# snarkify/sirius

Hardware: AMD Instinct MI355X
Metric: IVC fold-steps/s (CycleFold IVC::next hot path, Poseidon-shaped synthetic trace, 2^k rows) (higher is better)
Workload: dtype u256 (modular; 9 x 29-bit / 8 x 32-bit limbs)

## Files before the change

### sirius_amd/csrc/msm.h

```cpp
#pragma once
#include "curve.cuh"
#include "devrt.h"
#include "glv.cuh"
#include "stripes.h"
#include "tuning.h"

#include <cstdlib>

namespace srs {
namespace msm {

constexpr int WBITS = 16;
constexpr int NWIN = 16;
constexpr int NWIN_COMPACT = 8;
constexpr uint32_t PAY_ENDO = 1u << 30;
constexpr uint32_t NBUCKET = 1u << (WBITS - 1);

constexpr uint32_t SORT_THREADS = 1024;
constexpr uint32_t SORT_TILE_MIN = 8192;
constexpr uint32_t SORT_TARGET_BLOCKS = 256;
constexpr uint32_t SEG = 128, SEG_BUCKETS = NBUCKET / SEG;
constexpr uint32_t SORT_TILE2 = 8192;
constexpr uint64_t TWO_PASS_MIN_SLOTS = 1ull << 23;
constexpr uint32_t PLAN_THREADS = 1024;
constexpr uint32_t ACC_THREADS = 256;
constexpr uint32_t ACC_L0_LOG = 4, ACC_L0 = 1u << ACC_L0_LOG;
constexpr uint32_t ACC_L1_LOG = 3, ACC_L1 = 1u << ACC_L1_LOG;
constexpr uint32_t FINAL_THREADS = 256;
constexpr uint32_t FINAL_FANIN = 512;
constexpr int MAX_LEVELS = 8;
constexpr uint32_t RED_ROWS = 256;
constexpr uint32_t RED_COLS = NBUCKET / RED_ROWS;
constexpr uint32_t RED_THREADS = 4 * RED_COLS;
constexpr uint32_t ACC1_QUAD_MAX = 1u << 17;
constexpr uint32_t BATCH_ARGS = 16;
constexpr uint32_t LANDING_SLOTS = 16;
constexpr uint32_t NORM_G = 16;
constexpr uint32_t SLOT_LOG = 6;
constexpr uint32_t SLOT_L0_MIN_LOG = 2, SLOT_L0_MAX_LOG = 16;
constexpr int WBITS_W = 20;
constexpr int NWIN_W = 13;
constexpr uint32_t NSEG_W = 16;
constexpr uint32_t WIDE_THREADS = 256, WIDE_PER = 2, WIDE_TILE = WIDE_THREADS * WIDE_PER;
constexpr uint32_t WIDE_MIN_KEY_LOG = 23;
constexpr uint32_t WIDE_MIN_N_LOG = 23;

static_assert(RED_ROWS == 256 && RED_COLS == 128, "k_rowcol lane layout");
static_assert(NBUCKET % PLAN_THREADS == 0, "k_plan tiling");

inline bool expect_ovf_initial() { return tuning::get_or(tuning::MSM_EXPECT_OVF, 1) != 0; }

struct Key {
    int curve = 0;
    size_t len = 0;
    size_t global_len = 0;
    uint32_t rank = 0, world = 1;
    bool compact = false;
    bool compact_scalars = false;
    affine_t *table = nullptr;
    affine_t *table_w = nullptr;
    uint64_t stat_slot_sets = 0, stat_hot_sets = 0, stat_redo = 0, stat_other_sets = 0;
    uint64_t last_entries = 0;
    uint64_t last_scalars = 0;

    Arena arena;
    void *h_result = nullptr;
    struct Landing { bool wide = false, slot_mode = false, ovf_on = false; uint32_t batch = 0; } landing[LANDING_SLOTS];
    xyzz_t *fold_buckets = nullptr;
    xyzz_t *slots = nullptr;
    size_t slots_pts = 0;
    uint8_t *used = nullptr;
    uint32_t *h_ovf = nullptr;
    uint32_t slot_s = 0;
    uint32_t seq = 0;
    bool commit_ovf = false;
    bool expect_ovf = expect_ovf_initial();
    uint32_t cold_streak = 0;
};

int choose_windows(Key &k);
void build_table(Key &k, hipStream_t stream);
size_t table_bytes(const Key &k);
void release(Key &k);
void generate_bases(Key &k, uint64_t seed, hipStream_t stream);

void read_bases(const Key &k, affine_t *out_dev, hipStream_t stream);

size_t count_off_curve(const Key &k, hipStream_t stream);

size_t workspace_bytes(uint32_t n_max, uint32_t batch);

void run(Key &k, const fe_t *const *scalars_dev, const uint32_t *n_host, uint32_t batch, int is_mont,
         hipStream_t stream, xyzz_t *result_host);

enum Fold { FOLD_NONE = 0, FOLD_FIRST = 1, FOLD_MIDDLE = 2, FOLD_LAST = 3 };
bool enqueue(Key &k, const fe_t *const *scalars_dev, const uint32_t *n_host, const uint32_t *base_host, uint32_t batch, int is_mont,
             hipStream_t stream, uint32_t slot, Fold fold = FOLD_NONE);
void finish(Key &k, uint32_t batch, uint32_t slot, bool launched, xyzz_t *result_host);
void reserve(Key &k, uint32_t n_max, uint32_t batch);
bool overflow_missed(const Key &k, uint32_t slot);
void note_commit(Key &k, const uint32_t *slots_used, uint32_t n_slots, uint64_t scalars);

}
}
```

### sirius_amd/csrc/msm.hip

```cpp
#define SRS_F29_CHAIN 1
#include "msm.h"
#include "tuning.h"
#include "curve29.cuh"
#include "prof.h"

#include <algorithm>
#include <cstdlib>
#include <numeric>
#include <vector>

namespace srs {
namespace msm {

__device__ __forceinline__ uint32_t upper_bucket(const uint32_t *__restrict__ tp, uint32_t t) {
    uint32_t lo = 0, hi = NBUCKET;
    while (hi - lo > 1) {
        uint32_t mid = (lo + hi) >> 1;
        if (tp[mid] <= t) lo = mid; else hi = mid;
    }
    return lo;
}

template <class C>
__global__ void k_table_step(const affine_t *__restrict__ prev, xyzz_t *__restrict__ tmp, uint32_t n, int nbits) {
// ... 1381 lines not shown
    const size_t ping_off = link ? (size_t)link->base[0][m] : (size_t)m * ping_stride;
    const size_t pong_off = link ? (size_t)link->base[1][m] : (size_t)m * pong_stride;
    const xyzz_t *B = (hdr[1] && !from_buckets) ? ((hdr[0] & 1u) ? ping + ping_off : pong + pong_off) : buckets + (size_t)m * NBUCKET;
    using E29 = Ec29<C>;
    xyzz_t *out = rc + (size_t)m * (RED_ROWS + RED_COLS);
    const bool is_row = blockIdx.x < RED_ROWS / 2;
    xyzz29_t acc;
    if (is_row) {
        const uint32_t hi = blockIdx.x * 2 + wave;
        const xyzz_t *src = B + (size_t)hi * RED_COLS + vl * SER;
        acc = E29::unpack(src[0]);
        xyzz_t nx = src[1];
        for (uint32_t j = 1; j < SER; ++j) {
            xyzz_t cur = nx;
            if (j + 1 < SER) nx = src[j + 1];
            acc = E29::add_quad(acc, E29::unpack(cur), q);
        }
    } else {
        const uint32_t lo = blockIdx.x - RED_ROWS / 2, sub = wave * 16 + vl;
        const xyzz_t *src = B + (size_t)(sub * SER) * RED_COLS + lo;
        acc = E29::unpack(src[0]);
        xyzz_t nx = src[RED_COLS];
        for (uint32_t j = 1; j < SER; ++j) {
            xyzz_t cur = nx;
            if (j + 1 < SER) nx = src[(size_t)(j + 1) * RED_COLS];
            acc = E29::add_quad(acc, E29::unpack(cur), q);
        }
    }
    for (unsigned d = 8; d >= 1; d >>= 1) {
        xyzz29_t o = shfl_down_point29(acc, 4 * d, 64);
        if (vl < d) acc = E29::add_quad(acc, o, q);
    }
    if (is_row) {
        if (lane == 0) out[blockIdx.x * 2 + wave] = E29::pack(acc);
        return;
    }
    if (wave == 1 && lane == 0) half[0] = E29::pack(acc);
    __syncthreads();
    if (wave == 0 && vl == 0) {
        acc = E29::add_quad(acc, E29::unpack(half[0]), q);
        if (q == 0) out[RED_ROWS + (blockIdx.x - RED_ROWS / 2)] = E29::pack(acc);
    }
}

template <class C>
__global__ void SRS_KERNEL_BOUNDS(RED_THREADS, 1)
    k_reduce_final(const xyzz_t *__restrict__ rc, xyzz_t *__restrict__ out) {
    constexpr uint32_t N = RED_COLS;
    using E29 = Ec29<C>;
    __shared__ xyzz29_t v[N];
    const uint32_t m = blockIdx.y, t = threadIdx.x >> 2, q = threadIdx.x & 3u, which = blockIdx.x;
    const xyzz_t *rows = rc + (size_t)m * (RED_ROWS + RED_COLS), *cols = rows + RED_ROWS;
    xyzz29_t x;
    if (which == 0) x = E29::add_quad(E29::unpack(rows[2 * t]), E29::unpack(rows[2 * t + 1]), q);
    else if (which == 1 || which == 3) x = E29::unpack(cols[t]);
    else x = E29::unpack(rows[2 * t + 1]);
    if (which < 2) {
        if (q == 0) v[t] = x;
        __syncthreads();
        for (uint32_t s = 1; s < N; s <<= 1) {
            const bool has = t + s < N;
            xyzz29_t o = has ? v[t + s] : E29::identity();
            __syncthreads();
            if (has) x = E29::add_quad(x, o, q);
            if (q == 0) v[t] = x;
            __syncthreads();
        }
        if (which == 0 && t == 0) x = E29::identity();
    }
    if (q == 0) v[t] = x;
    __syncthreads();
    for (uint32_t s = N >> 1; s >= 1; s >>= 1) {
        if (t < s) {
            x = E29::add_quad(x, v[t + s], q);
            if (q == 0) v[t] = x;
        }
        __syncthreads();
    }
    if (threadIdx.x == 0) out[(size_t)m * gridDim.x + which] = E29::pack(v[0]);
}

template <class C>
__global__ void SRS_KERNEL_BOUNDS(256, 1)
    k_wide_combine(const xyzz_t *__restrict__ in , xyzz_t *__restrict__ out ) {
    using E29 = Ec29<C>;
    const uint32_t which = threadIdx.x >> 6, lane = threadIdx.x & 63u, q = lane & 3u, vl = lane >> 2;
    xyzz29_t x = E29::unpack(in[vl * 4 + which]);
    if (which == 3) {
        for (uint32_t s = 1; s < NSEG_W; s <<= 1) {
            xyzz29_t o = shfl_down_point29(x, 4 * s, 64);
            if (vl + s < NSEG_W) x = E29::add_quad(x, o, q);
        }
        if (vl == 0) x = E29::identity();
    }
    for (unsigned d = NSEG_W / 2; d >= 1; d >>= 1) {
        xyzz29_t o = shfl_down_point29(x, 4 * d, 64);
        if (vl < d) x = E29::add_quad(x, o, q);
    }
    if (lane == 0) out[which] = E29::pack(x);
}

static inline uint32_t ceil_div(uint64_t a, uint64_t b) { return (uint32_t)((a + b - 1) / b); }

template <class C>
static void expand_windows(affine_t *table, uint32_t n, int nwin, int nbits, xyzz_t *tmp, hipStream_t stream) {
    for (int w = 1; w < nwin; ++w) {
        const affine_t *prev = table + (size_t)(w - 1) * n;
        affine_t *cur = table + (size_t)w * n;
        SRS_LAUNCH((k_table_step<C>), (ceil_div(n, 256)), (256), 0, stream, prev, tmp, n, nbits);
        SRS_LAUNCH((k_normalize<C>), (ceil_div(ceil_div(n, NORM_G), 128)), (128), 0, stream, (const xyzz_t *)tmp, cur, n);
    }
}

static bool wants_wide_table(size_t len) {
    static const int env_forced = [] { const char *e = std::getenv("SRS_MSM_WIDE"); return e ? std::atoi(e) : -1; }();
    const int forced = (int)tuning::get_or(tuning::MSM_WIDE, env_forced);
    if (forced == 0 || len == 0) return false;
    return forced == 1 || len >= ((size_t)1 << WIDE_MIN_KEY_LOG);
}

template <class C>
static void build_table_t(Key &k, hipStream_t stream) {
    const uint32_t n = (uint32_t)k.len;
    if (k.table_w) {
        SRS_HIP_CHECK(hipFree(k.table_w));
        k.table_w = nullptr;
    }
    if (n == 0) return;
    xyzz_t *tmp = nullptr;
    SRS_HIP_CHECK(hipMalloc((void **)&tmp, (size_t)n * sizeof(xyzz_t)));
    if (!k.compact && wants_wide_table(n) && hipMalloc((void **)&k.table_w, (size_t)n * NWIN_W * sizeof(affine_t)) != hipSuccess) {
        (void)hipGetLastError();
        k.table_w = nullptr;
    }
    if (k.table_w) {
        SRS_HIP_CHECK(hipMemcpyAsync(k.table_w, k.table, (size_t)n * sizeof(affine_t), hipMemcpyDeviceToDevice, stream));
        expand_windows<C>(k.table_w, n, NWIN_W, WBITS_W, tmp, stream);
        const size_t total_w = (size_t)n * NWIN_W;
        SRS_LAUNCH((k_table_form<C>), (ceil_div(total_w, 256)), (256), 0, stream, k.table_w, total_w);
    }
    const int nwin = k.compact ? NWIN_COMPACT : NWIN;
    expand_windows<C>(k.table, n, nwin, WBITS, tmp, stream);
    const size_t total = (size_t)n * nwin;
    SRS_LAUNCH((k_table_form<C>), (ceil_div(total, 256)), (256), 0, stream, k.table, total);
    SRS_HIP_CHECK(hipStreamSynchronize(stream));
    SRS_HIP_CHECK(hipFree(tmp));
}

template <class C>
static void generate_t(Key &k, uint64_t seed, hipStream_t stream) {
    const uint32_t n = (uint32_t)k.len;
    if (n == 0) return;
    xyzz_t *tmp = nullptr;
    SRS_HIP_CHECK(hipMalloc((void **)&tmp, (size_t)n * sizeof(xyzz_t)));
    SRS_LAUNCH((k_gen_bases<C>), (ceil_div(n, 128)), (128), 0, stream, tmp, n, seed, k.rank, k.world);
    SRS_LAUNCH((k_normalize<C>), (ceil_div(ceil_div(n, NORM_G), 128)), (128), 0, stream, (const xyzz_t *)tmp, k.table, n);
    SRS_HIP_CHECK(hipStreamSynchronize(stream));
    SRS_HIP_CHECK(hipFree(tmp));
}
void generate_bases(Key &k, uint64_t seed, hipStream_t stream) {
    if (k.curve == 0) generate_t<Bn256>(k, seed, stream); else generate_t<Grumpkin>(k, seed, stream);
}

size_t count_off_curve(const Key &k, hipStream_t stream) {
    if (k.len == 0) return 0;
    uint32_t *d_bad = nullptr, bad = 0;
    SRS_HIP_CHECK(hipMalloc((void **)&d_bad, sizeof(uint32_t)));
    SRS_HIP_CHECK(hipMemsetAsync(d_bad, 0, sizeof(uint32_t), stream));
    const uint32_t n = (uint32_t)k.len;
    if (k.curve == 0) SRS_LAUNCH((k_on_curve<Bn256>), (ceil_div(n, 256)), (256), 0, stream, (const affine_t *)k.table, n, d_bad);
    else SRS_LAUNCH((k_on_curve<Grumpkin>), (ceil_div(n, 256)), (256), 0, stream, (const affine_t *)k.table, n, d_bad);
    SRS_HIP_CHECK(hipMemcpyAsync(&bad, d_bad, sizeof(uint32_t), hipMemcpyDeviceToHost, stream));
    SRS_HIP_CHECK(hipStreamSynchronize(stream));
    (void)hipFree(d_bad);
    return bad;
}

void read_bases(const Key &k, affine_t *out_dev, hipStream_t stream) {
    if (k.len == 0) return;
    if (k.curve == 0) SRS_LAUNCH((k_table_unform<Bn256>), (ceil_div(k.len, 256)), (256), 0, stream, (const affine_t *)k.table, out_dev, k.len);
    else SRS_LAUNCH((k_table_unform<Grumpkin>), (ceil_div(k.len, 256)), (256), 0, stream, (const affine_t *)k.table, out_dev, k.len);
}

void build_table(Key &k, hipStream_t stream) {
    if (k.curve == 0) build_table_t<Bn256>(k, stream); else build_table_t<Grumpkin>(k, stream);
}

int choose_windows(Key &k) {
    k.compact = tuning::get_or(tuning::MSM_COMPACT, 0) == 1;
    if (k.compact && (uint64_t)NWIN_COMPACT * k.len > PAY_ENDO) {
        set_error("compact key (msm_compact = 1): 8 x " + std::to_string(k.len) + " table entries do not fit below the endomorphism flag (2^30)");
        throw DeviceError{4};
    }
    return k.compact ? NWIN_COMPACT : NWIN;
}
size_t table_bytes(const Key &k) {
    if (!k.table) return 0;
    return k.len * sizeof(affine_t) * ((k.compact ? NWIN_COMPACT : NWIN) + (k.table_w ? NWIN_W : 0));
}


static uint32_t l0_log_for(uint64_t M) {
    const int forced = (int)tuning::get_or(tuning::MSM_L0, 0);
    if (forced >= 1 && forced <= 7) return (uint32_t)forced;
    if (M < (1ull << 20)) return 2;
    if (M < (1ull << 22)) return 3;
    uint32_t lg = ACC_L0_LOG;
    while (lg < 7 && (M >> (lg + 1)) >= (5ull << 20)) ++lg;
    return lg;
}

static uint32_t acc1_quad_max() {
    const int64_t lg = tuning::get_or(tuning::MSM_QUAD_MAX, 0);
    return (lg >= 1 && lg <= 24) ? (1u << lg) : ACC1_QUAD_MAX;
}

static int levels_for(uint64_t parts) {
    int levels = 1;
    while (parts > FINAL_FANIN && levels < MAX_LEVELS) {
        parts = (parts + ACC_L1 - 1) / ACC_L1;
        ++levels;
    }
    return levels;
}

static bool use_two_pass(uint64_t M, uint32_t batch) {
    const int forced = (int)tuning::get_or(tuning::MSM_SORT, 0);
    if (forced == 1) return false;
    if (forced == 2) return true;
    return M * batch >= TWO_PASS_MIN_SLOTS;
}

static uint32_t slot_log() {
    const int64_t lg = tuning::get_or(tuning::MSM_SLOT_LOG, 0);
    return (lg >= 2 && lg <= 8) ? (uint32_t)lg : SLOT_LOG;
}
static uint32_t slot_want_cap() { return 4u; }

struct LevelShape {
    uint64_t M;
    int levels;
    size_t plan_stride;
    uint64_t cap0, cap1;
    uint32_t quad_max;
};
struct SetShape : LevelShape {
    bool two_pass;
    uint32_t tile, tiles;
};
struct NarrowShape : SetShape { uint32_t l0_log; };
struct SlotShape : SetShape { uint32_t S, nred; };
struct WideShape : LevelShape { uint32_t l0_log, T, tiles_g; };

static void sort_shape(SetShape &h, uint32_t n_max, uint32_t batch) {
    h.M = (uint64_t)n_max * NWIN;
    h.quad_max = acc1_quad_max();
    h.two_pass = use_two_pass(h.M, batch);
    h.tile = (uint32_t)((h.M * batch + SORT_TARGET_BLOCKS - 1) / SORT_TARGET_BLOCKS);
    h.tile = (h.tile + 1023u) & ~1023u;
    if (h.tile < SORT_TILE_MIN) h.tile = SORT_TILE_MIN;
    h.tiles = ceil_div(n_max, h.tile);
}
static NarrowShape narrow_shape(uint32_t n_max, uint32_t batch) {
    NarrowShape h;
    sort_shape(h, n_max, batch);
    h.l0_log = l0_log_for(h.M);
    h.levels = levels_for((h.M + (1ull << h.l0_log) - 1) >> h.l0_log);
    h.plan_stride = (size_t)(h.levels + 1) * (NBUCKET + 1) + 4;
    h.cap0 = (h.M >> h.l0_log) + NBUCKET + 1;
    h.cap1 = h.cap0 / ACC_L1 + NBUCKET + 1;
    return h;
}
static SlotShape slot_shape(uint32_t n_max, uint32_t batch) {
    SlotShape h;
    sort_shape(h, n_max, batch);
    const uint32_t lg = slot_log();
    h.S = 1u << lg;
    h.nred = (lg + 2) / 3;
    h.cap0 = std::min<uint64_t>((uint64_t)NBUCKET * h.S, (h.M >> SLOT_L0_MIN_LOG) + NBUCKET);
    h.cap1 = h.cap0 / ACC_L1 + NBUCKET + 1;
    h.levels = levels_for(h.cap0);
    h.plan_stride = (size_t)(h.levels + 2) * (NBUCKET + 1) + 4;
    return h;
}
static WideShape wide_shape(uint32_t n) {
    WideShape w;
    w.M = (uint64_t)n * NWIN_W;
    w.quad_max = acc1_quad_max();
    w.l0_log = l0_log_for(w.M);
    w.levels = levels_for((w.M + (1ull << w.l0_log) - 1) >> w.l0_log);
    w.plan_stride = (size_t)(w.levels + 1) * (NBUCKET + 1) + 4;
    w.cap0 = (w.M >> w.l0_log) + (uint64_t)NSEG_W * (NBUCKET + 1);
    w.cap1 = w.cap0 / ACC_L1 + (uint64_t)NSEG_W * (NBUCKET + 1);
    w.T = ceil_div(n, WIDE_TILE);
    w.tiles_g = SORT_TARGET_BLOCKS;
    return w;
}

struct Sizer {
    size_t used = 0;
    template <class T>
    T *take(size_t count) {
        used += Arena::pad(count * sizeof(T));
        return nullptr;
    }
};
template <class Walk>
static size_t sized(Walk walk) {
    Sizer s;
    walk(s);
    return s.used;
}
template <class Walk>
static auto carve(Arena &A, Walk walk) {
    const size_t need = sized(walk);
    A.reserve(need);
    A.reset();
    const auto bufs = walk(A);
    if (A.used != need) {
        set_error("internal: msm workspace: the arena walk and the sizer disagree");
        throw DeviceError{5};
    }
    return bufs;
}

struct SetBufs {
    xyzz_t *d_out, *ping, *pong, *rc;
    uint16_t *dig, *tb;
    uint32_t *sorted, *count, *cursor, *plan;
    uint16_t *gkey;
    uint32_t *gpay, *tile_hist;
};
struct NarrowBufs : SetBufs { xyzz_t *buckets; };
struct SlotBufs : SetBufs { xyzz_t *red_a, *red_b; };
template <class W>
static void take_set_head(W &A, const SetShape &h, uint32_t batch, SetBufs &b) {
    b.d_out = A.template take<xyzz_t>(3 * (size_t)batch);
    b.dig = A.template take<uint16_t>(h.M * batch);
    b.sorted = A.template take<uint32_t>(h.M * batch);
    b.count = A.template take<uint32_t>((size_t)NBUCKET * batch);
    b.cursor = A.template take<uint32_t>((size_t)NBUCKET * batch);
    b.plan = A.template take<uint32_t>(h.plan_stride * batch);
    b.ping = A.template take<xyzz_t>(h.cap0 * batch);
    b.tb = A.template take<uint16_t>(h.cap0 * batch);
    b.pong = A.template take<xyzz_t>(h.cap1 * batch);
}
template <class W>
static void take_set_tail(W &A, const SetShape &h, uint32_t batch, SetBufs &b) {
    b.rc = A.template take<xyzz_t>((size_t)(RED_ROWS + RED_COLS) * batch);
    b.gkey = h.two_pass ? A.template take<uint16_t>(h.M * batch) : nullptr;
    b.gpay = h.two_pass ? A.template take<uint32_t>(h.M * batch) : nullptr;
    b.tile_hist = h.two_pass ? A.template take<uint32_t>((size_t)SEG * (SORT_TARGET_BLOCKS + 2 * NWIN) * batch) : nullptr;
}
template <class W>
static NarrowBufs narrow_layout(W &A, const NarrowShape &h, uint32_t batch) {
    NarrowBufs b;
    take_set_head(A, h, batch, b);
    b.buckets = A.template take<xyzz_t>((size_t)NBUCKET * batch);
    take_set_tail(A, h, batch, b);
    return b;
}
template <class W>
static SlotBufs slot_layout(W &A, const SlotShape &h, uint32_t batch) {
    SlotBufs b;
    take_set_head(A, h, batch, b);
    b.red_a = A.template take<xyzz_t>((size_t)NBUCKET * (h.S / 8 + 1) * batch);
    b.red_b = A.template take<xyzz_t>((size_t)NBUCKET * (h.S / 64 + 1) * batch);
    take_set_tail(A, h, batch, b);
    return b;
}
struct WideBufs {
    xyzz_t *d_out, *d_seg, *ping, *pong, *buckets, *rc;
    uint16_t *gkey, *gkey2, *tb;
    uint32_t *gpay, *gpay2, *tile_cnt, *tile_hist;
    uint32_t *seg3;
    uint32_t *sorted, *count, *cursor, *plan;
    Link *link;
};
template <class W>
static WideBufs wide_layout(W &A, const WideShape &w) {
    WideBufs b;
    b.d_out = A.template take<xyzz_t>(4);
    b.d_seg = A.template take<xyzz_t>(4 * NSEG_W);
    b.gkey = A.template take<uint16_t>(w.M);
    b.gpay = A.template take<uint32_t>(w.M);
    b.sorted = A.template take<uint32_t>(w.M);
    b.tile_cnt = A.template take<uint32_t>((size_t)NSEG_W * w.T);
    b.gkey2 = A.template take<uint16_t>(w.M);
    b.gpay2 = A.template take<uint32_t>(w.M);
    b.tile_hist = A.template take<uint32_t>((size_t)SEG * w.tiles_g);
    b.seg3 = A.template take<uint32_t>(4 * (NSEG_W + 2));
    b.link = A.template take<Link>(1);
    b.count = A.template take<uint32_t>((size_t)NSEG_W * NBUCKET);
    b.cursor = A.template take<uint32_t>((size_t)NSEG_W * NBUCKET);
    b.plan = A.template take<uint32_t>(w.plan_stride * NSEG_W);
    b.ping = A.template take<xyzz_t>(w.cap0);
    b.tb = A.template take<uint16_t>(w.cap0);
    b.pong = A.template take<xyzz_t>(w.cap1);
    b.buckets = A.template take<xyzz_t>((size_t)NSEG_W * NBUCKET);
    b.rc = A.template take<xyzz_t>((size_t)NSEG_W * (RED_ROWS + RED_COLS));
    return b;
}

size_t workspace_bytes(uint32_t n_max, uint32_t batch) {
    return sized([&](auto &A) { return narrow_layout(A, narrow_shape(n_max, batch), batch); });
}
static size_t workspace_bytes_slots(uint32_t n_max, uint32_t batch) {
    return sized([&](auto &A) { return slot_layout(A, slot_shape(n_max, batch), batch); });
}
static size_t workspace_bytes_wide(uint32_t n) {
    return sized([&](auto &A) { return wide_layout(A, wide_shape(n)); });
}

template <class C, class LaunchPlan>
static void sort_front(const Key &k, const SetShape &h, const SetBufs &b, const fe_t *const *scalars_dev, const uint32_t *n_host,
                       const uint32_t *base_host, uint32_t batch, uint32_t n_max, int is_mont, hipStream_t stream, LaunchPlan launch_plan,
                       bool group_maps, uint32_t arr) {
    BatchDesc bd;
    for (uint32_t m = 0; m < BATCH_ARGS; ++m) {
        bd.ptr[m] = m < batch ? scalars_dev[m] : nullptr;
        bd.n[m] = m < batch ? n_host[m] : 0;
        bd.base[m] = (m < batch && base_host) ? base_host[m] : 0;
    }
    const uint32_t s_rank = k.compact_scalars ? 0u : k.rank, s_world = k.compact_scalars ? 1u : k.world;
    const size_t M = (size_t)h.M;
    const auto digits = k.compact ? &k_digits<C, true> : &k_digits<C, false>;
    const auto group = k.compact ? &k_group<true> : &k_group<false>;
    const auto scatter = k.compact ? &k_scatter<true> : &k_scatter<false>;
    SRS_LAUNCH(digits, (ceil_div(n_max, 256), batch), (256), 0, stream, bd, b.dig, M, is_mont, s_rank, s_world, b.count,
               (uint32_t)(NBUCKET * batch));
    SRS_LAUNCH(k_hist, (h.tiles, NWIN, batch), (SORT_THREADS), 0, stream, (const uint16_t *)b.dig, M, bd, b.count, h.tile, b.tile_hist);
    launch_plan();
    if (h.two_pass) {
        const uint32_t T1 = h.tiles * NWIN;
        SRS_LAUNCH(k_scan_seg, (SEG, batch), (1024), 0, stream, b.tile_hist, T1, (const uint32_t *)b.plan, h.plan_stride);
        SRS_LAUNCH(group, (h.tiles, NWIN, batch), (SORT_THREADS), 0, stream, (const uint16_t *)b.dig, M, bd, (const uint32_t *)b.tile_hist,
                   b.gkey, b.gpay, M, (uint32_t)k.len, h.tile, group_maps ? (const uint32_t *)b.plan : nullptr,
                   group_maps ? h.plan_stride : (size_t)0, group_maps ? b.tb : nullptr, group_maps ? (size_t)h.cap0 : (size_t)0,
                   group_maps ? arr : 0u);
        SRS_LAUNCH(k_scatter2, (8 * ceil_div(ceil_div(M, SORT_TILE2), 8), batch), (SORT_THREADS), 0, stream, (const uint16_t *)b.gkey,
                   (const uint32_t *)b.gpay, M, (const uint32_t *)b.plan, h.plan_stride, b.cursor, b.sorted, M, (uint32_t)SORT_TILE2);
    } else {
        SRS_LAUNCH(scatter, (h.tiles, NWIN, batch), (SORT_THREADS), 0, stream, (const uint16_t *)b.dig, M, bd, b.cursor, b.sorted, M,
                   (uint32_t)k.len, h.tile);
    }
    if (!(h.two_pass && group_maps))
        SRS_LAUNCH(k_expand, (NBUCKET / 4, batch), (256), 0, stream, (const uint32_t *)b.plan, h.plan_stride, b.tb, (size_t)h.cap0,
                   (const Link *)nullptr, arr);
}

struct Parts {
    const uint32_t *plan; size_t plan_stride;
    xyzz_t *ping; size_t stride0;
    xyzz_t *pong; size_t stride1;
    const Link *link;
};

template <class C>
static void accum_levels(const Parts &p, const LevelShape &h, uint64_t cap_inc, uint32_t batch, hipStream_t stream) {
    xyzz_t *cur = p.ping, *nxt = p.pong;
    size_t cur_stride = p.stride0, nxt_stride = p.stride1;
    uint64_t cap = h.cap0;
    for (int level = 1; level < h.levels; ++level) {
        cap = cap / ACC_L1 + cap_inc;
        SRS_LAUNCH((k_accum1<C>), (ceil_div(std::max<uint64_t>(cap, 4 * std::min<uint64_t>(cap, h.quad_max)), ACC_THREADS), batch),
                   (ACC_THREADS), 0, stream, (const xyzz_t *)cur, cur_stride, p.plan, h.plan_stride, level, nxt, nxt_stride, (uint32_t)ACC_L1,
                   p.link, h.quad_max);
        std::swap(cur, nxt);
        std::swap(cur_stride, nxt_stride);
    }
}

template <class C>
static void reduce_buckets(const Parts &p, uint32_t nmsm, const xyzz_t *from, int from_buckets, xyzz_t *rc, uint32_t sums, xyzz_t *d_sums,
                           hipStream_t stream) {
    SRS_LAUNCH((k_rowcol<C>), (RED_ROWS / 2 + RED_COLS, nmsm), (128), 0, stream, from, (const xyzz_t *)p.ping, p.stride0,
               (const xyzz_t *)p.pong, p.stride1, p.plan, p.plan_stride, rc, p.link, from_buckets);
    SRS_LAUNCH((k_reduce_final<C>), (sums, nmsm), (RED_THREADS), 0, stream, (const xyzz_t *)rc, d_sums);
}

static void land(Key &k, const xyzz_t *d_out, size_t n, uint32_t slot, hipStream_t stream) {
    if (!k.h_result) SRS_HIP_CHECK(hipHostMalloc(&k.h_result, 3 * (size_t)BATCH_ARGS * LANDING_SLOTS * sizeof(xyzz_t)));
    xyzz_t *dst = static_cast<xyzz_t *>(k.h_result) + 3 * (size_t)BATCH_ARGS * slot;
    SRS_HIP_CHECK(hipMemcpyAsync(dst, d_out, n * sizeof(xyzz_t), hipMemcpyDeviceToHost, stream));
}

template <class C>
static bool enqueue_t(Key &k, const fe_t *const *scalars_dev, const uint32_t *n_host, const uint32_t *base_host, uint32_t batch,
                      uint32_t n_max, int is_mont, hipStream_t stream, uint32_t slot, Fold fold) {
    if (n_max == 0) return false;
    const NarrowShape h = narrow_shape(n_max, batch);
    const NarrowBufs b = carve(k.arena, [&](auto &A) { return narrow_layout(A, h, batch); });
    sort_front<C>(k, h, b, scalars_dev, n_host, base_host, batch, n_max, is_mont, stream, [&] {
        SRS_LAUNCH(k_plan, (batch, h.levels + 1), (PLAN_THREADS), 0, stream, (const uint32_t *)b.count, b.cursor, b.plan, h.plan_stride,
                   h.levels, h.l0_log, (uint32_t)ACC_L1_LOG, (const uint32_t *)nullptr);
    }, false, 1u);
    const Parts p{b.plan, h.plan_stride, b.ping, (size_t)h.cap0, b.pong, (size_t)h.cap1, nullptr};
    const uint64_t units = std::accumulate(n_host, n_host + batch, (uint64_t)0);
    const auto accum0 = k.compact ? &k_accum0c<C> : &k_accum0<C>;
    SRS_LAUNCH_TIMED("msm_accum0", units, accum0, (ceil_div(h.cap0, ACC_THREADS), batch), (ACC_THREADS), 0, stream,
                     (const uint32_t *)b.sorted, (size_t)h.M, p.plan, p.plan_stride, (const uint16_t *)b.tb, p.stride0,
                     (const affine_t *)k.table, p.ping, p.stride0, 1u << h.l0_log, p.link);
    accum_levels<C>(p, h, NBUCKET + 1, batch, stream);
    SRS_LAUNCH((k_accum_final<C>), (NBUCKET / (FINAL_THREADS / 64), batch), (FINAL_THREADS), 0, stream, (const xyzz_t *)p.ping, p.stride0,
               (const xyzz_t *)p.pong, p.stride1, p.plan, p.plan_stride, b.buckets, p.link);
    const xyzz_t *red_from = b.buckets;
    int from_buckets = 0;
    if (fold != FOLD_NONE) {
        if (!k.fold_buckets) SRS_HIP_CHECK(hipMalloc((void **)&k.fold_buckets, (size_t)NBUCKET * sizeof(xyzz_t)));
        SRS_LAUNCH((k_bucket_fold<C>), (NBUCKET / 64), (64), 0, stream, (const xyzz_t *)b.buckets, (const xyzz_t *)p.ping,
                   (const xyzz_t *)p.pong, p.plan, p.plan_stride, k.fold_buckets, fold == FOLD_FIRST ? 1 : 0);
        if (fold != FOLD_LAST) return true;
        red_from = k.fold_buckets;
        from_buckets = 1;
    }
    reduce_buckets<C>(p, batch, red_from, from_buckets, b.rc, 3, b.d_out, stream);
    land(k, b.d_out, 3 * (size_t)batch, slot, stream);
    k.landing[slot].wide = false;
    return true;
}

static bool use_wide(const Key &k, uint32_t n_max, uint32_t batch);
static bool use_slots(const Key &k, uint32_t n_max, uint32_t batch, Fold fold) {
    const int mode = (int)tuning::get_or(tuning::MSM_SLOTS, 1);
    if (mode == 0) return false;
    if (fold != FOLD_NONE) return batch == 1;
    return mode == 2 && !use_wide(k, n_max, batch);
}

template <class C>
static bool enqueue_slots_t(Key &k, const fe_t *const *scalars_dev, const uint32_t *n_host, const uint32_t *base_host, uint32_t batch,
                            uint32_t n_max, int is_mont, hipStream_t stream, uint32_t slot, Fold fold) {
    if (n_max == 0) return false;
    const bool first = fold == FOLD_NONE || fold == FOLD_FIRST, last = fold == FOLD_NONE || fold == FOLD_LAST;
    const SlotShape h = slot_shape(n_max, batch);
    const uint32_t S = h.S;
    if (first) {
        k.slot_s = S;
        k.seq = 0;
        k.commit_ovf = k.expect_ovf;
        const size_t need = (size_t)batch * NBUCKET * S;
        if (k.slots_pts < need) {
            if (k.slots) SRS_HIP_CHECK(hipFree(k.slots));
            k.slots = nullptr;
            k.slots_pts = 0;
            SRS_HIP_CHECK(hipMalloc((void **)&k.slots, need * sizeof(xyzz_t)));
            k.slots_pts = need;
        }
        if (!k.used) SRS_HIP_CHECK(hipMalloc((void **)&k.used, 2 * (size_t)BATCH_ARGS * NBUCKET));
        if (!k.h_ovf) {
            SRS_HIP_CHECK(hipHostMalloc((void **)&k.h_ovf, 2 * (size_t)LANDING_SLOTS * BATCH_ARGS * sizeof(uint32_t)));
            for (size_t i = 0; i < 2 * (size_t)LANDING_SLOTS * BATCH_ARGS; ++i) k.h_ovf[i] = 0;
        }
    } else if (k.slot_s != S || batch != 1) {
        set_error("internal: msm slot mode: a commit's sets must share the slot layout");
        throw DeviceError{5};
    }
    const uint8_t *used_prev = k.used + (size_t)(k.seq & 1u) * BATCH_ARGS * NBUCKET;
    uint8_t *used_next = k.used + (size_t)((k.seq + 1) & 1u) * BATCH_ARGS * NBUCKET;
    ++k.seq;

    const SlotBufs b = carve(k.arena, [&](auto &A) { return slot_layout(A, h, batch); });
    const uint32_t arr = (uint32_t)h.levels + 1;
    sort_front<C>(k, h, b, scalars_dev, n_host, base_host, batch, n_max, is_mont, stream, [&] {
        SRS_LAUNCH(k_plan_s, (batch, h.levels + 2), (PLAN_THREADS), 0, stream, (const uint32_t *)b.count, b.cursor, b.plan, h.plan_stride,
                   h.levels, S, (uint32_t)ACC_L1_LOG, used_prev, used_next, first ? 1 : 0, k.h_ovf + (size_t)slot * BATCH_ARGS, slot_want_cap());
    }, true, arr);
    const Parts p{b.plan, h.plan_stride, b.ping, (size_t)h.cap0, b.pong, (size_t)h.cap1, nullptr};
    const uint64_t units = std::accumulate(n_host, n_host + batch, (uint64_t)0);
    const auto accum0s = k.compact ? &k_accum0sc<C> : &k_accum0s<C>;
    SRS_LAUNCH_TIMED("msm_accum0", units, accum0s, (ceil_div(h.cap0, ACC_THREADS), batch), (ACC_THREADS), 0, stream,
                     (const uint32_t *)b.sorted, (size_t)h.M, p.plan, p.plan_stride, arr, (const uint16_t *)b.tb, p.stride0,
                     (const affine_t *)k.table, k.slots, S, used_prev, first ? 1 : 0, p.ping, p.stride0);
    if (k.commit_ovf) {
        accum_levels<C>(p, h, NBUCKET + 1, batch, stream);
        SRS_LAUNCH((k_ovf_final<C>), (NBUCKET / (FINAL_THREADS / 64), batch), (FINAL_THREADS), 0, stream, (const xyzz_t *)p.ping, p.stride0,
                   (const xyzz_t *)p.pong, p.stride1, p.plan, p.plan_stride, k.slots, S, first ? 1 : 0);
    }
    k.landing[slot] = {false, true, k.commit_ovf, batch};
    ++k.stat_slot_sets;
    if (!last) return true;
    const xyzz_t *in = k.slots;
    uint32_t in_pb = S;
    xyzz_t *outs[2] = {b.red_a, b.red_b};
    for (uint32_t l = 0; l < h.nred; ++l) {
        const uint32_t out_pb = (in_pb + 7) / 8, n_out = NBUCKET * out_pb;
        xyzz_t *out = outs[l & 1u];
        const uint8_t *used = l == 0 ? used_next : nullptr;
        const int extra = (l == 0 && k.commit_ovf) ? (int)S - 1 : -1;
        if (l + 1 == h.nred) {
            SRS_LAUNCH((k_slot_reduce<C, true>), (ceil_div((uint64_t)n_out * 4, 256), batch), (256), 0, stream, in, in_pb, used, (size_t)NBUCKET, extra,
                       out, out_pb);
        } else {
            SRS_LAUNCH((k_slot_reduce<C, false>), (ceil_div(n_out, 256), batch), (256), 0, stream, in, in_pb, used, (size_t)NBUCKET, extra, out,
                       out_pb);
        }
        in = out;
        in_pb = out_pb;
    }
    reduce_buckets<C>(p, batch, in, 1, b.rc, 3, b.d_out, stream);
    land(k, b.d_out, 3 * (size_t)batch, slot, stream);
    return true;
}

bool overflow_missed(const Key &k, uint32_t slot) {
    if (slot >= LANDING_SLOTS || !k.landing[slot].slot_mode || k.landing[slot].ovf_on || !k.h_ovf) return false;
    for (uint32_t m = 0; m < k.landing[slot].batch; ++m)
        if (k.h_ovf[(size_t)slot * BATCH_ARGS + m]) return true;
    return false;
}
void note_commit(Key &k, const uint32_t *slots_used, uint32_t n_slots, uint64_t scalars) {
    bool any = false, slot_sets = false;
    uint64_t entries = 0;
    for (uint32_t i = 0; i < n_slots; ++i) {
        const uint32_t sl = slots_used[i];
        if (sl >= LANDING_SLOTS || !k.landing[sl].slot_mode || !k.h_ovf) continue;
        slot_sets = true;
        for (uint32_t m = 0; m < k.landing[sl].batch; ++m) entries += k.h_ovf[(size_t)(LANDING_SLOTS + sl) * BATCH_ARGS + m];
        bool hot = false;
        for (uint32_t m = 0; m < k.landing[sl].batch; ++m) hot = hot || k.h_ovf[(size_t)sl * BATCH_ARGS + m] != 0;
        if (hot) ++k.stat_hot_sets;
        any = any || hot;
    }
    constexpr uint32_t COLD_COMMITS = 3;
    if (!slot_sets) {
        k.last_entries = k.last_scalars = 0;
        return;
    }
    k.last_entries = entries;
    k.last_scalars = scalars;
    if (any) {
        k.expect_ovf = true;
        k.cold_streak = 0;
    } else if (k.expect_ovf && ++k.cold_streak >= COLD_COMMITS) {
        k.expect_ovf = false;
        k.cold_streak = 0;
    }
}

static bool use_wide(const Key &k, uint32_t n_max, uint32_t batch) {
    const int min_log = (int)tuning::get_or(tuning::MSM_WIDE_MIN, (int64_t)WIDE_MIN_N_LOG);
    return k.table_w != nullptr && batch == 1 && n_max >= (1u << min_log);
}

template <class C>
static bool enqueue_wide_t(Key &k, const fe_t *scalars_dev, uint32_t n, uint32_t base, int is_mont, hipStream_t stream, uint32_t slot) {
    const WideShape w = wide_shape(n);
    const WideBufs b = carve(k.arena, [&](auto &A) { return wide_layout(A, w); });
    uint32_t *seg_total = b.seg3, *seg_off = b.seg3 + (NSEG_W + 2), *tile_base = b.seg3 + 2 * (NSEG_W + 2), *tile_base2 = b.seg3 + 3 * (NSEG_W + 2);

    WideDesc wd;
    wd.ptr = scalars_dev;
    wd.n = n;
    wd.base = base;
    wd.rank = k.compact_scalars ? 0u : k.rank;
    wd.world = k.compact_scalars ? 1u : k.world;
    wd.is_mont = is_mont;
    const uint32_t table_stride = (uint32_t)k.len;

    SRS_HIP_CHECK(hipMemsetAsync(seg_total, 0, (NSEG_W + 1) * sizeof(uint32_t), stream));
    SRS_HIP_CHECK(hipMemsetAsync(b.count, 0, (size_t)NSEG_W * NBUCKET * sizeof(uint32_t), stream));
    SRS_LAUNCH((k_seg_pass<C, false>), (w.T), (WIDE_THREADS), 0, stream, wd, b.tile_cnt, w.T, seg_total, (uint16_t *)nullptr,
               (uint32_t *)nullptr, table_stride);
    const uint32_t small_tiles = (w.M >> 19) < 64 ? 1u : 0u, tile2_host = small_tiles ? SORT_TILE2 / 4 : SORT_TILE2;
    SRS_LAUNCH(k_seg_scan, (NSEG_W), (1024), 0, stream, b.tile_cnt, w.T, (const uint32_t *)seg_total, seg_off, tile_base, tile_base2, small_tiles);
    SRS_LAUNCH((k_seg_pass<C, true>), (w.T), (WIDE_THREADS), 0, stream, wd, b.tile_cnt, w.T, seg_total, b.gkey, b.gpay, table_stride);
    SRS_LAUNCH(k_hist_g, (w.tiles_g), (SORT_THREADS), 0, stream, (const uint16_t *)b.gkey, (const uint32_t *)seg_off,
               (const uint32_t *)tile_base, b.count, b.tile_hist);
    SRS_LAUNCH(k_plan, (NSEG_W, w.levels + 1), (PLAN_THREADS), 0, stream, (const uint32_t *)b.count, b.cursor, b.plan, w.plan_stride, w.levels,
               w.l0_log, (uint32_t)ACC_L1_LOG, (const uint32_t *)seg_off);
    SRS_LAUNCH(k_scan_seg_g, (SEG, NSEG_W), (1024), 0, stream, b.tile_hist, w.tiles_g, (const uint32_t *)tile_base, (const uint32_t *)b.plan,
               w.plan_stride);
    SRS_LAUNCH(k_group_g, (w.tiles_g), (SORT_THREADS), 0, stream, (const uint16_t *)b.gkey, (const uint32_t *)b.gpay, (const uint32_t *)seg_off,
               (const uint32_t *)tile_base, (const uint32_t *)b.tile_hist, b.gkey2, b.gpay2);
    SRS_LAUNCH(k_scatter2_g, (8 * ceil_div(ceil_div(w.M, tile2_host) + NSEG_W, 8)), (SORT_THREADS), 0, stream, (const uint16_t *)b.gkey2,
               (const uint32_t *)b.gpay2, (const uint32_t *)seg_off, (const uint32_t *)tile_base2, b.cursor, b.sorted);
    SRS_LAUNCH(k_link, (1), (64), 0, stream, (const uint32_t *)b.plan, w.plan_stride, w.levels, b.link);
    const Parts p{b.plan, w.plan_stride, b.ping, 0, b.pong, 0, b.link};
    SRS_LAUNCH(k_expand, (NBUCKET / 4, NSEG_W), (256), 0, stream, p.plan, p.plan_stride, b.tb, (size_t)0, p.link, 1u);
    SRS_LAUNCH_TIMED("msm_accum0", n, (k_accum0<C>), (ceil_div(w.cap0, ACC_THREADS)), (ACC_THREADS), 0, stream, (const uint32_t *)b.sorted,
                     (size_t)0, p.plan, p.plan_stride, (const uint16_t *)b.tb, (size_t)0, (const affine_t *)k.table_w, p.ping, (size_t)0,
                     1u << w.l0_log, p.link);
    accum_levels<C>(p, w, (uint64_t)NSEG_W * (NBUCKET + 1), 1, stream);
    SRS_LAUNCH((k_accum_final<C>), (NBUCKET / (FINAL_THREADS / 64), NSEG_W), (FINAL_THREADS), 0, stream, (const xyzz_t *)p.ping, p.stride0,
               (const xyzz_t *)p.pong, p.stride1, p.plan, p.plan_stride, b.buckets, p.link);
    reduce_buckets<C>(p, NSEG_W, b.buckets, 0, b.rc, 4, b.d_seg, stream);
    SRS_LAUNCH((k_wide_combine<C>), (1), (256), 0, stream, (const xyzz_t *)b.d_seg, b.d_out);
    land(k, b.d_out, 4, slot, stream);
    k.landing[slot].wide = true;
    return true;
}

template <class C>
static void finish_t(Key &k, uint32_t batch, uint32_t slot, bool launched, xyzz_t *result_host) {
    if (!launched) {
        for (uint32_t m = 0; m < batch; ++m) result_host[m] = Ec<C>::identity();
        return;
    }
    const xyzz_t *raw = static_cast<const xyzz_t *>(k.h_result) + 3 * (size_t)BATCH_ARGS * slot;
    using F = typename C::F;
    fe_t c = F::one();
    for (int d = 0; d < 5; ++d) c = F::halve(c);
    std::vector<xyzz_t> two(3 * (size_t)batch + (k.landing[slot].wide ? 1 : 0));
    for (size_t i = 0; i < two.size(); ++i) {
        two[i].x = F::mul(raw[i].x, c);
        two[i].y = F::mul(raw[i].y, c);
        two[i].zz = F::mul(raw[i].zz, c);
        two[i].zzz = F::mul(raw[i].zzz, c);
    }
    for (uint32_t m = 0; m < batch; ++m) {
        xyzz_t a = Ec<C>::add(Ec<C>::dbl(two[3 * m]), two[3 * m + 2]);
        for (uint32_t j = 1; j < RED_COLS; j <<= 1) a = Ec<C>::dbl(a);
        result_host[m] = Ec<C>::add(a, two[3 * m + 1]);
    }
    if (k.landing[slot].wide) {
        xyzz_t u = two[3];
        for (uint32_t j = 1; j < NBUCKET; j <<= 1) u = Ec<C>::dbl(u);
        result_host[0] = Ec<C>::add(result_host[0], u);
    }
}

bool enqueue(Key &k, const fe_t *const *scalars_dev, const uint32_t *n_host, const uint32_t *base_host, uint32_t batch, int is_mont,
             hipStream_t stream, uint32_t slot, Fold fold) {
    if (batch > BATCH_ARGS || slot >= LANDING_SLOTS) {
        set_error("internal: msm::enqueue batch / slot out of range");
        throw DeviceError{5};
    }
    if (fold != FOLD_NONE && batch != 1) {
        set_error("internal: msm::enqueue fold needs one MSM per set");
        throw DeviceError{5};
    }
    if (batch == 1 && fold == FOLD_NONE && use_wide(k, n_host[0], 1)) {
        const uint32_t base = base_host ? base_host[0] : 0;
        k.landing[slot].slot_mode = false;
        ++k.stat_other_sets;
        return k.curve == 0 ? enqueue_wide_t<Bn256>(k, scalars_dev[0], n_host[0], base, is_mont, stream, slot)
                            : enqueue_wide_t<Grumpkin>(k, scalars_dev[0], n_host[0], base, is_mont, stream, slot);
    }
    uint32_t n_max = 0;
    for (uint32_t m = 0; m < batch; ++m) n_max = std::max(n_max, n_host[m]);
    const bool first = fold == FOLD_NONE || fold == FOLD_FIRST;
    const bool slots = first ? use_slots(k, n_max, batch, fold) : k.slot_s != 0;
    if (slots)
        return k.curve == 0 ? enqueue_slots_t<Bn256>(k, scalars_dev, n_host, base_host, batch, n_max, is_mont, stream, slot, fold)
                            : enqueue_slots_t<Grumpkin>(k, scalars_dev, n_host, base_host, batch, n_max, is_mont, stream, slot, fold);
    if (first) k.slot_s = 0;
    k.landing[slot].slot_mode = false;
    ++k.stat_other_sets;
    return k.curve == 0 ? enqueue_t<Bn256>(k, scalars_dev, n_host, base_host, batch, n_max, is_mont, stream, slot, fold)
                        : enqueue_t<Grumpkin>(k, scalars_dev, n_host, base_host, batch, n_max, is_mont, stream, slot, fold);
}
void finish(Key &k, uint32_t batch, uint32_t slot, bool launched, xyzz_t *result_host) {
    if (k.curve == 0) finish_t<Bn256>(k, batch, slot, launched, result_host); else finish_t<Grumpkin>(k, batch, slot, launched, result_host);
}
void reserve(Key &k, uint32_t n_max, uint32_t batch) {
    size_t b = use_wide(k, n_max, batch) ? std::max(workspace_bytes_wide(n_max), workspace_bytes(n_max, batch)) : workspace_bytes(n_max, batch);
    if (batch == 1) b = std::max(b, workspace_bytes_slots(n_max, batch));
    k.arena.reserve(b);
}

void release(Key &k) {
    if (k.table_w) (void)hipFree(k.table_w);
    k.table_w = nullptr;
    if (k.fold_buckets) (void)hipFree(k.fold_buckets);
    k.fold_buckets = nullptr;
    if (k.h_result) (void)hipHostFree(k.h_result);
    k.h_result = nullptr;
    if (k.slots) (void)hipFree(k.slots);
    k.slots = nullptr;
    k.slots_pts = 0;
    if (k.used) (void)hipFree(k.used);
    k.used = nullptr;
    if (k.h_ovf) (void)hipHostFree(k.h_ovf);
    k.h_ovf = nullptr;
    k.arena.release();
}

void run(Key &k, const fe_t *const *scalars_dev, const uint32_t *n_host, uint32_t batch, int is_mont,
         hipStream_t stream, xyzz_t *result_host) {
    for (uint32_t at = 0; at < batch;) {
        uint32_t b = std::min<uint32_t>(BATCH_ARGS, batch - at);
        if (use_wide(k, n_host[at], 1)) b = 1;
        bool launched = enqueue(k, scalars_dev + at, n_host + at, nullptr, b, is_mont, stream, 0);
        if (launched) {
            SRS_HIP_CHECK(hipStreamSynchronize(stream));
            SRS_HIP_CHECK(hipGetLastError());
            const uint32_t sl = 0;
            if (overflow_missed(k, sl)) {
                k.expect_ovf = true;
                ++k.stat_redo;
                launched = enqueue(k, scalars_dev + at, n_host + at, nullptr, b, is_mont, stream, 0);
                SRS_HIP_CHECK(hipStreamSynchronize(stream));
                SRS_HIP_CHECK(hipGetLastError());
            }
            uint64_t total = 0;
            for (uint32_t m = 0; m < b; ++m) total += n_host[at + m];
            note_commit(k, &sl, 1, total);
        }
        finish(k, b, 0, launched, result_host + at);
// ... 8 lines not shown
```

### sirius_amd/csrc/tuning.h

```cpp
#pragma once
#include <cstdint>

namespace srs {
namespace tuning {

enum Id : int {
    MSM_SORT = 0,
    MSM_L0,
    MSM_WIDE,
    MSM_WIDE_MIN,
    MSM_SLOTS,
    MSM_SLOT_LOG,
    MSM_EXPECT_OVF,
    MSM_QUAD_MAX,
    COMMIT_CHUNKS,
    PG_F_EVAL,
    PG_G_FFT,
    JIT_ALWAYS,
    NO_JIT,
    MSM_COMPACT,
    PG_COMPAT_TREE,
    N_TUNABLES
};

constexpr int64_t UNSET = INT64_MIN;

int64_t get(Id id);
inline int64_t get_or(Id id, int64_t dflt) {
    const int64_t v = get(id);
    return v == UNSET ? dflt : v;
}
int set(const char *name, int64_t value);
int64_t get_by_name(const char *name, int *found);
void reset();
const char *name_of(int id);

}
}
```

### sirius_amd/csrc/tuning.hip

```cpp
#include "tuning.h"

#include <atomic>
#include <cstring>

namespace srs {
namespace tuning {

static std::atomic<int64_t> g_val[N_TUNABLES];
static const char *const kNames[N_TUNABLES] = {"msm_sort", "msm_l0", "msm_wide", "msm_wide_min", "msm_slots", "msm_slot_log", "msm_expect_ovf",
                                               "msm_quad_max", "commit_chunks", "pg_f_eval", "pg_g_fft", "jit_always", "no_jit", "msm_compact", "pg_compat_tree"};
static struct Init {
    Init() { for (auto &v : g_val) v.store(UNSET, std::memory_order_relaxed); }
} g_init;

int64_t get(Id id) { return g_val[id].load(std::memory_order_relaxed); }
const char *name_of(int id) { return id >= 0 && id < N_TUNABLES ? kNames[id] : nullptr; }
static int find(const char *name) {
    if (!name) return -1;
    for (int i = 0; i < N_TUNABLES; ++i)
        if (std::strcmp(kNames[i], name) == 0) return i;
    return -1;
}
int set(const char *name, int64_t value) {
    const int i = find(name);
    if (i < 0) return -1;
    g_val[i].store(value, std::memory_order_relaxed);
    return 0;
}
int64_t get_by_name(const char *name, int *found) {
    const int i = find(name);
    if (found) *found = i >= 0;
    return i < 0 ? UNSET : get((Id)i);
}
void reset() { for (auto &v : g_val) v.store(UNSET, std::memory_order_relaxed); }

}
}
```

Before: 99.69.

## Split MSM bucket row/column reduction into 16x16 partial sums finished on host

Adds a k_reduce_split kernel that reduces the 256 row sums and 128 column sums as 16-wide blocks with per-block weighting. It emits four partial points instead of three, and the host recombines them with a few extra doublings. This removes the long serial prefix chain in k_reduce_final, which used RED_THREADS blocks with a deep running sum, in favour of shallower shuffle trees across more small blocks. It is on by default through a new msm_reduce_split tunable. Landing buffers, the wide-combine kernel and the host finish code are widened to carry the extra sum.

```diff
diff --git a/sirius_amd/csrc/msm.h b/sirius_amd/csrc/msm.h
--- a/sirius_amd/csrc/msm.h
+++ b/sirius_amd/csrc/msm.h
@@ -32,9 +32,12 @@
 constexpr uint32_t RED_ROWS = 256;
 constexpr uint32_t RED_COLS = NBUCKET / RED_ROWS;
 constexpr uint32_t RED_THREADS = 4 * RED_COLS;
+constexpr uint32_t RED_SPLIT = 16;
+constexpr uint32_t RED_SUMS_MAX = 4;
 constexpr uint32_t ACC1_QUAD_MAX = 1u << 17;
 constexpr uint32_t BATCH_ARGS = 16;
 constexpr uint32_t LANDING_SLOTS = 16;
+constexpr size_t LANDING_POINTS = (size_t)RED_SUMS_MAX * BATCH_ARGS;
 constexpr uint32_t NORM_G = 16;
 constexpr uint32_t SLOT_LOG = 6;
 constexpr uint32_t SLOT_L0_MIN_LOG = 2, SLOT_L0_MAX_LOG = 16;
@@ -65,7 +68,7 @@
 
     Arena arena;
     void *h_result = nullptr;
-    struct Landing { bool wide = false, slot_mode = false, ovf_on = false; uint32_t batch = 0; } landing[LANDING_SLOTS];
+    struct Landing { bool wide = false, slot_mode = false, ovf_on = false; uint32_t batch = 0; bool split = false; } landing[LANDING_SLOTS];
     xyzz_t *fold_buckets = nullptr;
     xyzz_t *slots = nullptr;
     size_t slots_pts = 0;
diff --git a/sirius_amd/csrc/msm.hip b/sirius_amd/csrc/msm.hip
--- a/sirius_amd/csrc/msm.hip
+++ b/sirius_amd/csrc/msm.hip
@@ -1487,11 +1487,52 @@
 
 template <class C>
 __global__ void SRS_KERNEL_BOUNDS(256, 1)
+    k_reduce_split(const xyzz_t *__restrict__ rc, xyzz_t *__restrict__ out) {
+    static_assert(RED_ROWS == RED_SPLIT * RED_SPLIT && RED_COLS == RED_SPLIT * (RED_SPLIT / 2), "k_reduce_split: 16 x 16 row sums, 8 x 16 column sums");
+    using E29 = Ec29<C>;
+    __shared__ xyzz29_t g[RED_SPLIT];
+    const uint32_t m = blockIdx.y, which = blockIdx.x, t = threadIdx.x >> 2, q = threadIdx.x & 3u;
+    const xyzz_t *in = rc + (size_t)m * (RED_ROWS + RED_COLS) + (which < 2 ? 0u : RED_ROWS);
+    const uint32_t U = which == 2 ? RED_SPLIT / 2 : RED_SPLIT;
+    const uint32_t V = (which < 2 ? RED_ROWS : RED_COLS) / U;
+    const bool u_high = which == 0 || which == 2;
+    const uint32_t qpo = 64 / U, ser = V / qpo;
+    const uint32_t u = t / qpo, sub = t % qpo;
+    xyzz29_t x = E29::identity();
+    for (uint32_t j = 0; j < ser; ++j) {
+        const uint32_t v = sub * ser + j;
+        const xyzz29_t y = E29::unpack(in[u_high ? V * u + v : U * v + u]);
+        x = j == 0 ? y : E29::add_quad(x, y, q);
+    }
+    for (uint32_t d = qpo >> 1; d >= 1; d >>= 1) {
+        xyzz29_t o = shfl_down_point29(x, 4 * d, 64);
+        if (sub < d) x = E29::add_quad(x, o, q);
+    }
+    if (sub == 0 && q == 0) g[u] = x;
+    __syncthreads();
+    if (threadIdx.x >= 64) return;
+    x = t < U ? g[t] : E29::identity();
+    if (which < 4) {
+        for (uint32_t s = 1; s < U; s <<= 1) {
+            xyzz29_t o = shfl_down_point29(x, 4 * s, 64);
+            if (t + s < U) x = E29::add_quad(x, o, q);
+        }
+        if (which != 3 && t == 0) x = E29::identity();
+    }
+    for (uint32_t d = RED_SPLIT >> 1; d >= 1; d >>= 1) {
+        xyzz29_t o = shfl_down_point29(x, 4 * d, 64);
+        if (t < d) x = E29::add_quad(x, o, q);
+    }
+    if (threadIdx.x == 0) out[(size_t)m * gridDim.x + which] = E29::pack(x);
+}
+
+template <class C>
+__global__ void SRS_KERNEL_BOUNDS(64 * (RED_SUMS_MAX + 1), 1)
     k_wide_combine(const xyzz_t *__restrict__ in , xyzz_t *__restrict__ out ) {
     using E29 = Ec29<C>;
-    const uint32_t which = threadIdx.x >> 6, lane = threadIdx.x & 63u, q = lane & 3u, vl = lane >> 2;
-    xyzz29_t x = E29::unpack(in[vl * 4 + which]);
-    if (which == 3) {
+    const uint32_t nsum = blockDim.x >> 6, which = threadIdx.x >> 6, lane = threadIdx.x & 63u, q = lane & 3u, vl = lane >> 2;
+    xyzz29_t x = E29::unpack(in[vl * nsum + which]);
+    if (which == nsum - 1) {
         for (uint32_t s = 1; s < NSEG_W; s <<= 1) {
             xyzz29_t o = shfl_down_point29(x, 4 * s, 64);
             if (vl + s < NSEG_W) x = E29::add_quad(x, o, q);
@@ -1636,6 +1677,9 @@
     return M * batch >= TWO_PASS_MIN_SLOTS;
 }
 
+static constexpr uint32_t red_sums(bool split) { return split ? 4u : 3u; }
+static bool reduce_split() { return tuning::get_or(tuning::MSM_REDUCE_SPLIT, 1) != 0; }
+
 static uint32_t slot_log() {
     const int64_t lg = tuning::get_or(tuning::MSM_SLOT_LOG, 0);
     return (lg >= 2 && lg <= 8) ? (uint32_t)lg : SLOT_LOG;
@@ -1648,6 +1692,7 @@
     size_t plan_stride;
     uint64_t cap0, cap1;
     uint32_t quad_max;
+    bool split;
 };
 struct SetShape : LevelShape {
     bool two_pass;
@@ -1660,6 +1705,7 @@
 static void sort_shape(SetShape &h, uint32_t n_max, uint32_t batch) {
     h.M = (uint64_t)n_max * NWIN;
     h.quad_max = acc1_quad_max();
+    h.split = reduce_split();
     h.two_pass = use_two_pass(h.M, batch);
     h.tile = (uint32_t)((h.M * batch + SORT_TARGET_BLOCKS - 1) / SORT_TARGET_BLOCKS);
     h.tile = (h.tile + 1023u) & ~1023u;
@@ -1692,6 +1738,7 @@
     WideShape w;
     w.M = (uint64_t)n * NWIN_W;
     w.quad_max = acc1_quad_max();
+    w.split = reduce_split();
     w.l0_log = l0_log_for(w.M);
     w.levels = levels_for((w.M + (1ull << w.l0_log) - 1) >> w.l0_log);
     w.plan_stride = (size_t)(w.levels + 1) * (NBUCKET + 1) + 4;
@@ -1740,7 +1787,7 @@
 struct SlotBufs : SetBufs { xyzz_t *red_a, *red_b; };
 template <class W>
 static void take_set_head(W &A, const SetShape &h, uint32_t batch, SetBufs &b) {
-    b.d_out = A.template take<xyzz_t>(3 * (size_t)batch);
+    b.d_out = A.template take<xyzz_t>(RED_SUMS_MAX * (size_t)batch);
     b.dig = A.template take<uint16_t>(h.M * batch);
     b.sorted = A.template take<uint32_t>(h.M * batch);
     b.count = A.template take<uint32_t>((size_t)NBUCKET * batch);
@@ -1785,8 +1832,8 @@
 template <class W>
 static WideBufs wide_layout(W &A, const WideShape &w) {
     WideBufs b;
-    b.d_out = A.template take<xyzz_t>(4);
-    b.d_seg = A.template take<xyzz_t>(4 * NSEG_W);
+    b.d_out = A.template take<xyzz_t>(RED_SUMS_MAX + 1);
+    b.d_seg = A.template take<xyzz_t>((RED_SUMS_MAX + 1) * NSEG_W);
     b.gkey = A.template take<uint16_t>(w.M);
     b.gpay = A.template take<uint32_t>(w.M);
     b.sorted = A.template take<uint32_t>(w.M);
@@ -1877,16 +1924,19 @@
 }
 
 template <class C>
-static void reduce_buckets(const Parts &p, uint32_t nmsm, const xyzz_t *from, int from_buckets, xyzz_t *rc, uint32_t sums, xyzz_t *d_sums,
-                           hipStream_t stream) {
+static void reduce_buckets(const Parts &p, uint32_t nmsm, const xyzz_t *from, int from_buckets, xyzz_t *rc, bool split, bool total,
+                           xyzz_t *d_sums, hipStream_t stream) {
     SRS_LAUNCH((k_rowcol<C>), (RED_ROWS / 2 + RED_COLS, nmsm), (128), 0, stream, from, (const xyzz_t *)p.ping, p.stride0,
                (const xyzz_t *)p.pong, p.stride1, p.plan, p.plan_stride, rc, p.link, from_buckets);
-    SRS_LAUNCH((k_reduce_final<C>), (sums, nmsm), (RED_THREADS), 0, stream, (const xyzz_t *)rc, d_sums);
+    if (split)
+        SRS_LAUNCH((k_reduce_split<C>), (red_sums(true) + (total ? 1 : 0), nmsm), (256), 0, stream, (const xyzz_t *)rc, d_sums);
+    else
+        SRS_LAUNCH((k_reduce_final<C>), (red_sums(false) + (total ? 1 : 0), nmsm), (RED_THREADS), 0, stream, (const xyzz_t *)rc, d_sums);
 }
 
 static void land(Key &k, const xyzz_t *d_out, size_t n, uint32_t slot, hipStream_t stream) {
-    if (!k.h_result) SRS_HIP_CHECK(hipHostMalloc(&k.h_result, 3 * (size_t)BATCH_ARGS * LANDING_SLOTS * sizeof(xyzz_t)));
-    xyzz_t *dst = static_cast<xyzz_t *>(k.h_result) + 3 * (size_t)BATCH_ARGS * slot;
+    if (!k.h_result) SRS_HIP_CHECK(hipHostMalloc(&k.h_result, LANDING_POINTS * LANDING_SLOTS * sizeof(xyzz_t)));
+    xyzz_t *dst = static_cast<xyzz_t *>(k.h_result) + LANDING_POINTS * slot;
     SRS_HIP_CHECK(hipMemcpyAsync(dst, d_out, n * sizeof(xyzz_t), hipMemcpyDeviceToHost, stream));
 }
 
@@ -1919,9 +1969,10 @@
         red_from = k.fold_buckets;
         from_buckets = 1;
     }
-    reduce_buckets<C>(p, batch, red_from, from_buckets, b.rc, 3, b.d_out, stream);
-    land(k, b.d_out, 3 * (size_t)batch, slot, stream);
+    reduce_buckets<C>(p, batch, red_from, from_buckets, b.rc, h.split, false, b.d_out, stream);
+    land(k, b.d_out, red_sums(h.split) * (size_t)batch, slot, stream);
     k.landing[slot].wide = false;
+    k.landing[slot].split = h.split;
     return true;
 }
 
@@ -1982,7 +2033,7 @@
         SRS_LAUNCH((k_ovf_final<C>), (NBUCKET / (FINAL_THREADS / 64), batch), (FINAL_THREADS), 0, stream, (const xyzz_t *)p.ping, p.stride0,
                    (const xyzz_t *)p.pong, p.stride1, p.plan, p.plan_stride, k.slots, S, first ? 1 : 0);
     }
-    k.landing[slot] = {false, true, k.commit_ovf, batch};
+    k.landing[slot] = {false, true, k.commit_ovf, batch, h.split};
     ++k.stat_slot_sets;
     if (!last) return true;
     const xyzz_t *in = k.slots;
@@ -2003,8 +2054,8 @@
         in = out;
         in_pb = out_pb;
     }
-    reduce_buckets<C>(p, batch, in, 1, b.rc, 3, b.d_out, stream);
-    land(k, b.d_out, 3 * (size_t)batch, slot, stream);
+    reduce_buckets<C>(p, batch, in, 1, b.rc, h.split, false, b.d_out, stream);
+    land(k, b.d_out, red_sums(h.split) * (size_t)batch, slot, stream);
     return true;
 }
 
@@ -2089,10 +2140,12 @@
     accum_levels<C>(p, w, (uint64_t)NSEG_W * (NBUCKET + 1), 1, stream);
     SRS_LAUNCH((k_accum_final<C>), (NBUCKET / (FINAL_THREADS / 64), NSEG_W), (FINAL_THREADS), 0, stream, (const xyzz_t *)p.ping, p.stride0,
                (const xyzz_t *)p.pong, p.stride1, p.plan, p.plan_stride, b.buckets, p.link);
-    reduce_buckets<C>(p, NSEG_W, b.buckets, 0, b.rc, 4, b.d_seg, stream);
-    SRS_LAUNCH((k_wide_combine<C>), (1), (256), 0, stream, (const xyzz_t *)b.d_seg, b.d_out);
-    land(k, b.d_out, 4, slot, stream);
+    const uint32_t nsum = red_sums(w.split) + 1;
+    reduce_buckets<C>(p, NSEG_W, b.buckets, 0, b.rc, w.split, true, b.d_seg, stream);
+    SRS_LAUNCH((k_wide_combine<C>), (1), (64 * nsum), 0, stream, (const xyzz_t *)b.d_seg, b.d_out);
+    land(k, b.d_out, nsum, slot, stream);
     k.landing[slot].wide = true;
+    k.landing[slot].split = w.split;
     return true;
 }
 
@@ -2102,11 +2155,13 @@
         for (uint32_t m = 0; m < batch; ++m) result_host[m] = Ec<C>::identity();
         return;
     }
-    const xyzz_t *raw = static_cast<const xyzz_t *>(k.h_result) + 3 * (size_t)BATCH_ARGS * slot;
+    const xyzz_t *raw = static_cast<const xyzz_t *>(k.h_result) + LANDING_POINTS * slot;
+    const bool split = k.landing[slot].split;
+    const uint32_t ns = red_sums(split);
     using F = typename C::F;
     fe_t c = F::one();
     for (int d = 0; d < 5; ++d) c = F::halve(c);
-    std::vector<xyzz_t> two(3 * (size_t)batch + (k.landing[slot].wide ? 1 : 0));
+    std::vector<xyzz_t> two(ns * (size_t)batch + (k.landing[slot].wide ? 1 : 0));
     for (size_t i = 0; i < two.size(); ++i) {
         two[i].x = F::mul(raw[i].x, c);
         two[i].y = F::mul(raw[i].y, c);
@@ -2114,12 +2169,22 @@
         two[i].zzz = F::mul(raw[i].zzz, c);
     }
     for (uint32_t m = 0; m < batch; ++m) {
+        if (split) {
+            xyzz_t a = two[4 * m];
+            for (uint32_t j = 1; j < RED_SPLIT; j <<= 1) a = Ec<C>::dbl(a);
+            a = Ec<C>::add(a, two[4 * m + 1]);
+            for (uint32_t j = 1; j < RED_COLS / RED_SPLIT; j <<= 1) a = Ec<C>::dbl(a);
+            a = Ec<C>::add(a, two[4 * m + 2]);
+            for (uint32_t j = 1; j < RED_SPLIT; j <<= 1) a = Ec<C>::dbl(a);
+            result_host[m] = Ec<C>::add(a, two[4 * m + 3]);
+            continue;
+        }
         xyzz_t a = Ec<C>::add(Ec<C>::dbl(two[3 * m]), two[3 * m + 2]);
         for (uint32_t j = 1; j < RED_COLS; j <<= 1) a = Ec<C>::dbl(a);
         result_host[m] = Ec<C>::add(a, two[3 * m + 1]);
     }
     if (k.landing[slot].wide) {
-        xyzz_t u = two[3];
+        xyzz_t u = two[ns];
         for (uint32_t j = 1; j < NBUCKET; j <<= 1) u = Ec<C>::dbl(u);
         result_host[0] = Ec<C>::add(result_host[0], u);
     }
diff --git a/sirius_amd/csrc/tuning.h b/sirius_amd/csrc/tuning.h
--- a/sirius_amd/csrc/tuning.h
+++ b/sirius_amd/csrc/tuning.h
@@ -20,6 +20,7 @@
     NO_JIT,
     MSM_COMPACT,
     PG_COMPAT_TREE,
+    MSM_REDUCE_SPLIT,
     N_TUNABLES
 };
 
diff --git a/sirius_amd/csrc/tuning.hip b/sirius_amd/csrc/tuning.hip
--- a/sirius_amd/csrc/tuning.hip
+++ b/sirius_amd/csrc/tuning.hip
@@ -8,7 +8,8 @@
 
 static std::atomic<int64_t> g_val[N_TUNABLES];
 static const char *const kNames[N_TUNABLES] = {"msm_sort", "msm_l0", "msm_wide", "msm_wide_min", "msm_slots", "msm_slot_log", "msm_expect_ovf",
-                                               "msm_quad_max", "commit_chunks", "pg_f_eval", "pg_g_fft", "jit_always", "no_jit", "msm_compact", "pg_compat_tree"};
+                                               "msm_quad_max", "commit_chunks", "pg_f_eval", "pg_g_fft", "jit_always", "no_jit", "msm_compact", "pg_compat_tree",
+                                               "msm_reduce_split"};
 static struct Init {
     Init() { for (auto &v : g_val) v.store(UNSET, std::memory_order_relaxed); }
 } g_init;
```

Result: no change. 99.46 (-0.2%).
